# liamhebert/MultiModalDiscussionTransformer

Measured on AMD Instinct MI355X. Metric: discussion-tree comments/sec fwd+bwd, higher is better.
Workload: dtype bf16; 1 GPU; mDT-base (BERT-base + ViT-B/16 split 6+6, 6 executed graph layers, D768 H12 nb4 L100), 32 bushy 64-comment trees per GPU, 25% image comments, random-init weights, dropout 0.4/0.3/0.3 (run_train.sh:37), token lengths U{8..100} zero-padded to 100 (SURVEY.md §8d; mean 54.3 valid tokens), text side ragged: padded token positions are not computed (identical logits / gradients), last fusion layer comput; trees_per_gpu=32, parallelism=dp1, frozen_initial_encoders=False

## Files before the change

multimodaldiscussiontransformer_amd/csrc/common.hpp:

```cpp
#pragma once
#include <hip/hip_runtime.h>
#include <stdint.h>
#include <stdio.h>
#include <string.h>

#include <atomic>

#include "../../include/mdt_hip.h"

namespace mdt {

constexpr int WAVE = 64;

typedef __bf16 bf16_t;
typedef __attribute__((ext_vector_type(8))) __bf16 bf16x8;
typedef __attribute__((ext_vector_type(4))) __bf16 bf16x4;
typedef __attribute__((ext_vector_type(2))) __bf16 bf16x2;
typedef __attribute__((ext_vector_type(4))) float f32x4;
typedef __attribute__((ext_vector_type(2))) float f32x2;
typedef __attribute__((ext_vector_type(4))) short s16x4;
typedef __attribute__((ext_vector_type(4))) int i32x4;

void set_error(const char* fmt, ...);
#define MDT_CHECK_ARG(cond, ...)          \
  do {                                    \
    if (!(cond)) {                        \
      ::mdt::set_error(__VA_ARGS__);      \
      return MDT_ERR_ARG;                 \
    }                                     \
  } while (0)
#define MDT_UNSUPPORTED(...)              \
  do {                                    \
    ::mdt::set_error(__VA_ARGS__);        \
    return MDT_ERR_UNSUPPORTED;           \
  } while (0)
int check_launch(const char* what);

enum class GemmRoute { none, generic, tile128, tile256x128, pp256, pp256p, w4p, w4s };
inline constexpr const char* GEMM_ROUTE_NAMES[] = {"", "generic", "tile128", "tile256x128", "pp256", "pp256p", "w4p", "w4s"};
enum class AttnRoute { none, v1, v2, v3, v4, v4x, v5, long_ };
inline constexpr const char* ATTN_ROUTE_NAMES[] = {"", "v1", "v2", "v3", "v4", "v4x", "v5", "long"};
inline const char* route_name(GemmRoute r) { return GEMM_ROUTE_NAMES[(int)r]; }
inline const char* route_name(AttnRoute r) { return ATTN_ROUTE_NAMES[(int)r]; }

struct Switches {
  GemmRoute gemm_route;
  bool gemm_dynamic;
  bool gemm_stamp;
  int gemm_diag;
  int gemm_f8w;
  AttnRoute attn_bwd;
  bool ln_generic;
  int ln_bwd_wgs;
};
const Switches& switches();
int device_cus();

void set_last_route(const char* route);
template <auto Kern, typename... Args>
int launch_route(const char* route, dim3 grid, dim3 block, size_t lds, hipStream_t st, Args... args) {
  static std::atomic<size_t> raised{64 * 1024};
  if (lds > raised.load(std::memory_order_relaxed)) {
    if (hipFuncSetAttribute((const void*)Kern, hipFuncAttributeMaxDynamicSharedMemorySize, (int)lds) != hipSuccess) {
      (void)hipGetLastError();
      set_error("%s: cannot reserve %zu bytes of LDS", route, lds);
      return MDT_ERR_LAUNCH;
    }
    raised.store(lds, std::memory_order_relaxed);
  }
  hipLaunchKernelGGL(Kern, grid, block, lds, st, args...);
  if (int e = check_launch(route)) return e;
  set_last_route(route);
  return MDT_OK;
}

template <typename T> __device__ __forceinline__ float to_f32(T v);
template <> __device__ __forceinline__ float to_f32<float>(float v) { return v; }
template <> __device__ __forceinline__ float to_f32<bf16_t>(bf16_t v) { return (float)v; }
template <typename T> __device__ __forceinline__ T from_f32(float v);
template <> __device__ __forceinline__ float from_f32<float>(float v) { return v; }
template <> __device__ __forceinline__ bf16_t from_f32<bf16_t>(float v) { return (bf16_t)v; }

__device__ __forceinline__ float wave_sum(float v) {
#pragma unroll
  for (int o = 32; o > 0; o >>= 1) v += __shfl_xor(v, o, 64);
  return v;
}
__device__ __forceinline__ float wave_max(float v) {
#pragma unroll
  for (int o = 32; o > 0; o >>= 1) v = fmaxf(v, __shfl_xor(v, o, 64));
  return v;
}
__device__ __forceinline__ float quad16_sum(float v) {
  v += __shfl_xor(v, 16, 64);
  v += __shfl_xor(v, 32, 64);
  return v;
}
__device__ __forceinline__ float row16_sum(float v) {
#pragma unroll
  for (int o = 8; o > 0; o >>= 1) v += __shfl_xor(v, o, 64);
  return v;
}
__device__ __forceinline__ float row16_sum_dpp(float v) {
  v += __builtin_bit_cast(float, __builtin_amdgcn_mov_dpp(__builtin_bit_cast(int, v), 0x128, 0xf, 0xf, true));
  v += __builtin_bit_cast(float, __builtin_amdgcn_mov_dpp(__builtin_bit_cast(int, v), 0x124, 0xf, 0xf, true));
  v += __builtin_bit_cast(float, __builtin_amdgcn_mov_dpp(__builtin_bit_cast(int, v), 0x122, 0xf, 0xf, true));
  v += __builtin_bit_cast(float, __builtin_amdgcn_mov_dpp(__builtin_bit_cast(int, v), 0x121, 0xf, 0xf, true));
  return v;
}
__device__ __forceinline__ float wave_sum_dpp(float v) {
  v = row16_sum_dpp(v);
  v += __builtin_bit_cast(float, __builtin_amdgcn_update_dpp(0, __builtin_bit_cast(int, v), 0x142, 0xa, 0xf, false));
  v += __builtin_bit_cast(float, __builtin_amdgcn_update_dpp(0, __builtin_bit_cast(int, v), 0x143, 0xc, 0xf, false));
  return __builtin_bit_cast(float, __builtin_amdgcn_readlane(__builtin_bit_cast(int, v), 63));
}
__device__ __forceinline__ float row16_max(float v) {
#pragma unroll
  for (int o = 8; o > 0; o >>= 1) v = fmaxf(v, __shfl_xor(v, o, 64));
  return v;
}

__device__ __forceinline__ float gelu_erf(float x) { return 0.5f * x * (1.0f + erff(x * 0.70710678118654752f)); }
__device__ __forceinline__ float gelu_erf_grad(float x) {
  const float cdf = 0.5f * (1.0f + erff(x * 0.70710678118654752f));
  const float pdf = 0.3989422804014327f * __expf(-0.5f * x * x);
  return cdf + x * pdf;
}

__device__ __forceinline__ void gelu_fast_parts(float x, float& cdf, float& pdf) {
  const float z = fabsf(x) * 0.70710678118654752f;
  const float t = __builtin_amdgcn_rcpf(__builtin_fmaf(0.3275911f, z, 1.0f));
  const float e = __builtin_amdgcn_exp2f(z * z * -1.4426950408889634f);
  float poly = __builtin_fmaf(t, 1.061405429f, -1.453152027f);
  poly = __builtin_fmaf(t, poly, 1.421413741f);
  poly = __builtin_fmaf(t, poly, -0.284496736f);
  poly = __builtin_fmaf(t, poly, 0.254829592f);
  const float erf_abs = __builtin_fmaf(-(poly * t), e, 1.0f);
  cdf = __builtin_fmaf(0.5f, copysignf(erf_abs, x), 0.5f);
  pdf = 0.3989422804014327f * e;
}
__device__ __forceinline__ float gelu_fast(float x) {
  float cdf, pdf;
  gelu_fast_parts(x, cdf, pdf);
  return x * cdf;
}
__device__ __forceinline__ float gelu_fast_grad(float x) {
  float cdf, pdf;
  gelu_fast_parts(x, cdf, pdf);
  return cdf + x * pdf;
}

__device__ __forceinline__ uint32_t drop_mix(uint32_t x) {
  x = __umul24(x, 0x95F24Du) + __builtin_rotateleft32(x, 15); x ^= x >> 15;
  x = __umul24(x, 0xC2B2AEu) + __builtin_rotateleft32(x, 13); x ^= x >> 13;
  x = __umul24(x, 0x85EBCBu) + __builtin_rotateleft32(x, 17); x ^= x >> 16;
  return x;
}
struct DropCfg {
  uint32_t key;
  uint32_t thresh;
  float inv_keep;
};
__device__ __forceinline__ float drop_scale(const DropCfg& d, uint64_t idx) {
  const uint32_t h = drop_mix((uint32_t)(idx >> 1) ^ d.key);
  const uint32_t bits = (idx & 1) ? (h >> 16) : (h & 0xFFFFu);
  return bits >= d.thresh ? d.inv_keep : 0.f;
}
__device__ __forceinline__ void drop_scale2(const DropCfg& d, uint64_t idx_even, float& s0, float& s1) {
  const uint32_t h = drop_mix((uint32_t)(idx_even >> 1) ^ d.key);
  s0 = (h & 0xFFFFu) >= d.thresh ? d.inv_keep : 0.f;
  s1 = (h >> 16) >= d.thresh ? d.inv_keep : 0.f;
}
constexpr int64_t DROP_MAX_ELEMS = (int64_t)1 << 33;
static inline DropCfg make_drop(float p, uint64_t seed) {
  DropCfg d;
  uint64_t z = seed + 0x9E3779B97F4A7C15ull;
  z = (z ^ (z >> 30)) * 0xBF58476D1CE4E5B9ull;
  z = (z ^ (z >> 27)) * 0x94D049BB133111EBull;
  z ^= z >> 31;
  d.key = (uint32_t)(z ^ (z >> 32));
  d.thresh = (uint32_t)(p * 65536.0f + 0.5f);
  d.inv_keep = 1.0f / (1.0f - p);
  return d;
}

__device__ __forceinline__ f32x4 mfma_f32(float a, float b, f32x4 c) {
  return __builtin_amdgcn_mfma_f32_16x16x4f32(a, b, c, 0, 0, 0);
}
__device__ __forceinline__ f32x4 mfma_bf16(bf16x8 a, bf16x8 b, f32x4 c) {
  return __builtin_amdgcn_mfma_f32_16x16x32_bf16(a, b, c, 0, 0, 0);
}

#define LDS_PTR(p) ((__attribute__((address_space(3))) void*)(p))

__device__ __forceinline__ bf16x4 lds_read_tr16(const bf16_t* lds_addr) {
  typedef __attribute__((address_space(3))) s16x4* lds_s16x4_ptr;
  s16x4 r = __builtin_amdgcn_ds_read_tr16_b64_v4i16((lds_s16x4_ptr)(lds_addr));
  return __builtin_bit_cast(bf16x4, r);
}

__device__ __forceinline__ void glds16(const void* gptr, void* lds_wave_base) {
  __builtin_amdgcn_global_load_lds((const __attribute__((address_space(1))) void*)gptr,
// ... 11 lines not shown
```

multimodaldiscussiontransformer_amd/csrc/gemm.hip:

```cpp
#include <stdlib.h>

#include <algorithm>
#include <type_traits>
#include <vector>

#include "common.hpp"
#include "gemm_tiles.hpp"
#include "gemm_epilogue.hpp"

namespace mdt {

template <typename TIn, typename TOut, bool TA, bool TB>
__global__ __launch_bounds__(256) void gemm_generic_kernel(GemmParams p) {
  constexpr int BM = 64, BN = 64, BK = 16, LD = 68;
  __shared__ float As[BK][LD];
  __shared__ float Bs[BK][LD];
  const int tid = threadIdx.x, lane = tid & 63, wave = tid >> 6;
  const int wr = wave >> 1, wc = wave & 1;
  const int64_t m0 = (int64_t)blockIdx.y * BM, n0 = (int64_t)blockIdx.x * BN;
  const int64_t kbeg = (int64_t)blockIdx.z * p.k_chunk;
  const int64_t kend = (kbeg + p.k_chunk < p.K) ? kbeg + p.k_chunk : p.K;
  const TIn* A = (const TIn*)p.A;
  const TIn* B = (const TIn*)p.B;
  f32x4 acc[2][2];
#pragma unroll
  for (int i = 0; i < 2; ++i)
#pragma unroll
    for (int j = 0; j < 2; ++j) acc[i][j] = f32x4{0.f, 0.f, 0.f, 0.f};

  for (int64_t k0 = kbeg; k0 < kend; k0 += BK) {
#pragma unroll
    for (int i = 0; i < 4; ++i) {
      const int e = tid + i * 256;
      int r, k;
      if constexpr (!TA) { r = e >> 4; k = e & 15; } else { k = e >> 6; r = e & 63; }
      const int64_t gr = m0 + r, gk = k0 + k;
      float v = 0.f;
      if (gr < p.M && gk < kend) v = to_f32(TA ? A[gk * p.lda + gr] : A[gr * p.lda + gk]);
      As[k][r] = v;
      int c, kb;
      if constexpr (!TB) { c = e >> 4; kb = e & 15; } else { kb = e >> 6; c = e & 63; }
      const int64_t gc = n0 + c, gkb = k0 + kb;
      float w = 0.f;
      if (gc < p.N && gkb < kend) w = to_f32(TB ? B[gkb * p.ldb + gc] : B[gc * p.ldb + gkb]);
      Bs[kb][c] = w;
    }
    __syncthreads();
#pragma unroll
    for (int kk = 0; kk < BK; kk += 4) {
      float a[2], b[2];
#pragma unroll
      for (int i = 0; i < 2; ++i) a[i] = As[kk + (lane >> 4)][wr * 32 + i * 16 + (lane & 15)];
#pragma unroll
      for (int j = 0; j < 2; ++j) b[j] = Bs[kk + (lane >> 4)][wc * 32 + j * 16 + (lane & 15)];
#pragma unroll
      for (int i = 0; i < 2; ++i)
#pragma unroll
        for (int j = 0; j < 2; ++j) acc[i][j] = mfma_f32(a[i], b[j], acc[i][j]);
    }
    __syncthreads();
  }
#pragma unroll
  for (int i = 0; i < 2; ++i)
#pragma unroll
    for (int j = 0; j < 2; ++j)
#pragma unroll
      for (int r = 0; r < 4; ++r)
        epilogue_store<TIn, TOut>(p, m0 + wr * 32 + i * 16 + (lane >> 4) * 4 + r,
                                  n0 + wc * 32 + j * 16 + (lane & 15), acc[i][j][r]);
}

template <typename TOut, bool A_KM, bool B_KM>
__global__ __launch_bounds__(256) void gemm_bf16_tile128(GemmParams p) {
  extern __shared__ __attribute__((aligned(16))) char smem[];
  const int tid = threadIdx.x;
  const int lane = tid & 63;
  const int wave = __builtin_amdgcn_readfirstlane(tid >> 6);
  const int wr = wave >> 1, wc = wave & 1;

  const int nwg = p.tiles_m * p.tiles_n;
  const int bid = blockIdx.x;
  const int q8 = nwg >> 3, r8 = nwg & 7, xcd = bid & 7;
  const int tile = (xcd < r8 ? xcd * (q8 + 1) : r8 * (q8 + 1) + (xcd - r8) * q8) + (bid >> 3);
  const int tm = tile / p.tiles_n, tn = tile - tm * p.tiles_n;
  const int64_t m0 = (int64_t)tm * T_BM, n0 = (int64_t)tn * T_BN;
  const int64_t kbeg = (int64_t)blockIdx.z * p.k_chunk;
  const int64_t kend = (kbeg + p.k_chunk < p.K) ? kbeg + p.k_chunk : p.K;
  const int nk = (int)((kend - kbeg + T_BK - 1) / T_BK);

  const int64_t lda_b = p.lda * 2, ldb_b = p.ldb * 2;
  const char* a_base;
  const char* b_base;
  int64_t a_bytes, b_bytes;
  if constexpr (!A_KM) { a_base = (const char*)p.A + m0 * lda_b; a_bytes = (p.M - m0) * lda_b; }
  else { a_base = (const char*)p.A + kbeg * lda_b; a_bytes = (kend - kbeg) * lda_b; }
  if constexpr (!B_KM) { b_base = (const char*)p.B + n0 * ldb_b; b_bytes = (p.N - n0) * ldb_b; }
  else { b_base = (const char*)p.B + kbeg * ldb_b; b_bytes = (kend - kbeg) * ldb_b; }
  const unsigned a_rec = (unsigned)(a_bytes > 0xFFFFFFF0ll ? 0xFFFFFFF0ll : a_bytes);
  const unsigned b_rec = (unsigned)(b_bytes > 0xFFFFFFF0ll ? 0xFFFFFFF0ll : b_bytes);
  const __amdgpu_buffer_rsrc_t rsA = __builtin_amdgcn_make_buffer_rsrc((void*)a_base, 0, a_rec, 0x00020000);
  const __amdgpu_buffer_rsrc_t rsB = __builtin_amdgcn_make_buffer_rsrc((void*)b_base, 0, b_rec, 0x00020000);
  const int64_t a_k0 = A_KM ? 0 : kbeg, b_k0 = B_KM ? 0 : kbeg;
  const int a_col0 = A_KM ? (int)m0 : 0, b_col0 = B_KM ? (int)n0 : 0;

  f32x4 acc[4][4];
#pragma unroll
  for (int i = 0; i < 4; ++i)
#pragma unroll
    for (int j = 0; j < 4; ++j) acc[i][j] = f32x4{0.f, 0.f, 0.f, 0.f};

  if (nk > 0) {
    stage_tile<A_KM, 128, 4>(rsA, lda_b, a_k0, a_col0, smem, wave, lane);
    stage_tile<B_KM, 128, 4>(rsB, ldb_b, b_k0, b_col0, smem + T_TILE_BYTES, wave, lane);
  }
  for (int kt = 0; kt < nk; ++kt) {
    char* cur = smem + (kt & 1) * 2 * T_TILE_BYTES;
    char* nxt = smem + ((kt + 1) & 1) * 2 * T_TILE_BYTES;
    __syncthreads();
    if (kt + 1 < nk) {
      stage_tile<A_KM, 128, 4>(rsA, lda_b, a_k0 + (int64_t)(kt + 1) * T_BK, a_col0, nxt, wave, lane);
      stage_tile<B_KM, 128, 4>(rsB, ldb_b, b_k0 + (int64_t)(kt + 1) * T_BK, b_col0, nxt + T_TILE_BYTES, wave, lane);
    }
#pragma unroll
    for (int ks = 0; ks < 2; ++ks) {
      bf16x8 a[4], b[4];
#pragma unroll
      for (int i = 0; i < 4; ++i) a[i] = load_frag<A_KM, 128>(cur, wr * 64 + i * 16, ks, lane);
#pragma unroll
      for (int j = 0; j < 4; ++j) b[j] = load_frag<B_KM, 128>(cur + T_TILE_BYTES, wc * 64 + j * 16, ks, lane);
#pragma unroll
      for (int i = 0; i < 4; ++i)
#pragma unroll
        for (int j = 0; j < 4; ++j) acc[i][j] = mfma_bf16(a[i], b[j], acc[i][j]);
    }
  }
  tile_epilogue<TOut>(p, acc, smem, wave, lane, m0 + wr * 64, n0 + wc * 64);
}

template <typename TOut, bool A_KM, bool B_KM, int BN, int WM, int WN, int NSTAGE>
__global__ __launch_bounds__(512) void gemm_bf16_tile256(GemmParams p) {
  constexpr int BM = 256;
  constexpr int MI = BM / WM / 16, NI = BN / WN / 16;
  constexpr int A_BYTES = BM * 128, B_BYTES = BN * 128, STAGE = A_BYTES + B_BYTES;
  constexpr int LOADS = (BM + BN) / 64;
  extern __shared__ __attribute__((aligned(16))) char smem[];
  const int tid = threadIdx.x;
  const int lane = tid & 63;
  const int wave = __builtin_amdgcn_readfirstlane(tid >> 6);
  const int wr = wave / WN, wc = wave % WN;

  const int nwg = p.tiles_m * p.tiles_n;
  const int bid = blockIdx.x;
  const int q8 = nwg >> 3, r8 = nwg & 7, xcd = bid & 7;
  const int tile = (xcd < r8 ? xcd * (q8 + 1) : r8 * (q8 + 1) + (xcd - r8) * q8) + (bid >> 3);
  const int tm = tile / p.tiles_n, tn = tile - tm * p.tiles_n;
  const int64_t m0 = (int64_t)tm * BM, n0 = (int64_t)tn * BN;
  const int64_t kbeg = (int64_t)blockIdx.z * p.k_chunk;
  const int64_t kend = (kbeg + p.k_chunk < p.K) ? kbeg + p.k_chunk : p.K;
  const int nk = (int)((kend - kbeg + T_BK - 1) / T_BK);

  const int64_t lda_b = p.lda * 2, ldb_b = p.ldb * 2;
  const char* a_base;
  const char* b_base;
  int64_t a_bytes, b_bytes;
  if constexpr (!A_KM) { a_base = (const char*)p.A + m0 * lda_b; a_bytes = (p.M - m0) * lda_b; }
  else { a_base = (const char*)p.A + kbeg * lda_b; a_bytes = (kend - kbeg) * lda_b; }
  if constexpr (!B_KM) { b_base = (const char*)p.B + n0 * ldb_b; b_bytes = (p.N - n0) * ldb_b; }
  else { b_base = (const char*)p.B + kbeg * ldb_b; b_bytes = (kend - kbeg) * ldb_b; }
  const unsigned a_rec = (unsigned)(a_bytes > 0xFFFFFFF0ll ? 0xFFFFFFF0ll : a_bytes);
  const unsigned b_rec = (unsigned)(b_bytes > 0xFFFFFFF0ll ? 0xFFFFFFF0ll : b_bytes);
  const __amdgpu_buffer_rsrc_t rsA = __builtin_amdgcn_make_buffer_rsrc((void*)a_base, 0, a_rec, 0x00020000);
  const __amdgpu_buffer_rsrc_t rsB = __builtin_amdgcn_make_buffer_rsrc((void*)b_base, 0, b_rec, 0x00020000);
  const int64_t a_k0 = A_KM ? 0 : kbeg, b_k0 = B_KM ? 0 : kbeg;
  const int a_col0 = A_KM ? (int)m0 : 0, b_col0 = B_KM ? (int)n0 : 0;

  f32x4 acc[MI][NI];
#pragma unroll
  for (int i = 0; i < MI; ++i)
#pragma unroll
    for (int j = 0; j < NI; ++j) acc[i][j] = f32x4{0.f, 0.f, 0.f, 0.f};

  auto issue = [&](int kt) {
    char* st = smem + (kt % NSTAGE) * STAGE;
    stage_tile<A_KM, BM, 8>(rsA, lda_b, a_k0 + (int64_t)kt * T_BK, a_col0, st, wave, lane);
    stage_tile<B_KM, BN, 8>(rsB, ldb_b, b_k0 + (int64_t)kt * T_BK, b_col0, st + A_BYTES, wave, lane);
  };
#pragma unroll
  for (int s = 0; s < NSTAGE - 1; ++s)
    if (nk > s) issue(s);
  for (int kt = 0; kt < nk; ++kt) {
    if (NSTAGE == 3 && kt + 1 < nk) {
      if constexpr (LOADS == 6) asm volatile("s_waitcnt vmcnt(6)" ::: "memory");
      else asm volatile("s_waitcnt vmcnt(8)" ::: "memory");
    } else {
      asm volatile("s_waitcnt vmcnt(0)" ::: "memory");
    }
    __builtin_amdgcn_s_barrier();
    if (kt + NSTAGE - 1 < nk) issue(kt + NSTAGE - 1);
    const char* cur = smem + (kt % NSTAGE) * STAGE;
#pragma unroll
    for (int ks = 0; ks < 2; ++ks) {
      bf16x8 a[MI], b[NI];
#pragma unroll
      for (int j = 0; j < NI; ++j) b[j] = load_frag<B_KM, BN>(cur + A_BYTES, wc * (NI * 16) + j * 16, ks, lane);
#pragma unroll
      for (int i = 0; i < MI; ++i) a[i] = load_frag<A_KM, BM>(cur, wr * (MI * 16) + i * 16, ks, lane);
#pragma unroll
      for (int i = 0; i < MI; ++i)
#pragma unroll
        for (int j = 0; j < NI; ++j) acc[i][j] = mfma_bf16(a[i], b[j], acc[i][j]);
    }
  }
#pragma unroll
  for (int h = 0; h < MI / 4; ++h) {
    f32x4 blk[4][4];
#pragma unroll
    for (int i = 0; i < 4; ++i)
#pragma unroll
      for (int j = 0; j < 4; ++j) blk[i][j] = acc[h * 4 + i][j];
    tile_epilogue<TOut>(p, blk, smem, wave, lane, m0 + wr * (MI * 16) + h * 64, n0 + wc * 64);
  }
}

constexpr int pp_nb(int dist) { return dist + 1 < 4 ? 4 : dist + 1; }

template <typename TOut, bool A_KM, bool B_KM, int PP_DIST>
__global__ __launch_bounds__(512) void gemm_bf16_pp256(GemmParams p) {
  constexpr int PP_NB = pp_nb(PP_DIST);
  constexpr int BM = 256, BN = 256;
  constexpr int A_BYTES = BM * 64;
  constexpr bool SWAP = sizeof(TOut) == 2;
  extern __shared__ __attribute__((aligned(16))) char smem[];
  const int tid = threadIdx.x;
  const int lane = tid & 63;
  const int wave = __builtin_amdgcn_readfirstlane(tid >> 6);
  const int wr = wave >> 2, wc = wave & 3;
  const bool late = wave >= 4;

  const int tiles = p.tiles_m * p.tiles_n;
  const int nwg = tiles * (int)gridDim.z;
  const int bid = (int)blockIdx.z * (int)gridDim.x + (int)blockIdx.x;
  const int q8 = nwg >> 3, r8 = nwg & 7, xcd = bid & 7;
  const int work = (xcd < r8 ? xcd * (q8 + 1) : r8 * (q8 + 1) + (xcd - r8) * q8) + (bid >> 3);
  const int slab = work / tiles;
  const int tile = work - slab * tiles;
  int tm, tn;
  {
    const int G = p.group_n, per_group = p.tiles_m * G;
    const int gi = tile / per_group;
    const int full = p.tiles_n / G;
    if (gi < full) {
      const int r = tile - gi * per_group;
      tm = r / G;
      tn = gi * G + (r - tm * G);
    } else {
      const int gsz = p.tiles_n - full * G;
      const int r = tile - full * per_group;
      tm = r / gsz;
      tn = full * G + (r - tm * gsz);
    }
  }
  const int64_t m0 = (int64_t)tm * BM, n0 = (int64_t)tn * BN;
  const int64_t kbeg = (int64_t)slab * p.k_chunk;
  const int64_t kend = (kbeg + p.k_chunk < p.K) ? kbeg + p.k_chunk : p.K;
  const int nk = (int)((kend - kbeg + T_BK - 1) / T_BK);
  const int nhs = 2 * nk;

  const int64_t lda_b = p.lda * 2, ldb_b = p.ldb * 2;
  const char* a_base;
  const char* b_base;
  int64_t a_bytes, b_bytes;
  if constexpr (!A_KM) { a_base = (const char*)p.A + m0 * lda_b; a_bytes = (p.M - m0) * lda_b; }
  else { a_base = (const char*)p.A + kbeg * lda_b; a_bytes = (kend - kbeg) * lda_b; }
  if constexpr (!B_KM) { b_base = (const char*)p.B + n0 * ldb_b; b_bytes = (p.N - n0) * ldb_b; }
  else { b_base = (const char*)p.B + kbeg * ldb_b; b_bytes = (kend - kbeg) * ldb_b; }
  const unsigned a_rec = (unsigned)(a_bytes > 0xFFFFFFF0ll ? 0xFFFFFFF0ll : a_bytes);
  const unsigned b_rec = (unsigned)(b_bytes > 0xFFFFFFF0ll ? 0xFFFFFFF0ll : b_bytes);
  const __amdgpu_buffer_rsrc_t rsA = __builtin_amdgcn_make_buffer_rsrc((void*)a_base, 0, a_rec, 0x00020000);
  const __amdgpu_buffer_rsrc_t rsB = __builtin_amdgcn_make_buffer_rsrc((void*)b_base, 0, b_rec, 0x00020000);
  const int64_t a_k0 = A_KM ? 0 : kbeg, b_k0 = B_KM ? 0 : kbeg;
  const int a_col0 = A_KM ? (int)m0 : 0, b_col0 = B_KM ? (int)n0 : 0;

  f32x4 acc[8][4];
#pragma unroll
  for (int i = 0; i < 8; ++i)
#pragma unroll
    for (int j = 0; j < 4; ++j) acc[i][j] = f32x4{0.f, 0.f, 0.f, 0.f};
// ... 704 lines not shown
  std::sort(cyc.begin(), cyc.end());
  std::sort(clk.begin(), clk.end());
  fprintf(stderr, "[mdt gemm stamp] M=%lld N=%lld K=%lld wgs=%zu  cycles/k-tile median %.0f (p10 %.0f p90 %.0f)  clock median %.0f MHz  span %.1f us\n",
          (long long)p.M, (long long)p.N, (long long)p.K, nwg, cyc[cyc.size() / 2], cyc[cyc.size() / 10], cyc[cyc.size() * 9 / 10],
          clk[clk.size() / 2], (double)(t1 - t0) / 100.0);
  std::vector<unsigned long long> st(256);
  if (hipMemcpy(st.data(), dev + nwg * 4, 256 * 8, hipMemcpyDeviceToHost) == hipSuccess && st[0]) {
    fprintf(stderr, "[mdt gemm steps]");
    for (int i = 1; i < 256 && st[i]; ++i) fprintf(stderr, " %llu", st[i] - st[i - 1]);
    fprintf(stderr, "\n");
  } else (void)hipGetLastError();
}

static int num_cus() {
  const int n = device_cus() & ~7;
  return n < 8 ? 8 : n;
}

static int* g_tile_queues = nullptr;
static int g_tile_queue_sets = 0;

static int xcd_group_n(int tiles_m, int tiles_n, double b_panel, int n_cus) {
  if (tiles_n % 2 == 0 && b_panel * tiles_n > 3.5e6 && b_panel * (tiles_n / 2) <= 2.5e6 && (double)tiles_m * tiles_n >= 4.0 * n_cus)
    return tiles_n / 2;
  return tiles_n;
}

struct GemmPlan {
  GemmRoute route;
  int tiles_m, tiles_n, split_k, group_n;
  int64_t k_chunk;
  dim3 grid;
  bool strip_asum;
};

static GemmPlan plan_gemm(const GemmParams& p, int dtype, int out_dtype, int ta, int tb, int n_cus) {
  const Switches& sw = switches();
  const int64_t M = p.M, N = p.N, K = p.K;
  const int epi = p.epilogue;
  bool fast = dtype == MDT_BF16 && K > 0 && (ta ? M % T_BM == 0 : K % T_BK == 0) && (tb ? N % T_BN == 0 : K % T_BK == 0) &&
              N % T_BN == 0 && p.lda % 8 == 0 && p.ldb % 8 == 0 && ((uintptr_t)p.A | (uintptr_t)p.B) % 16 == 0 &&
              p.lda * 2 * 128 < (1ll << 31) && p.ldb * 2 * 128 < (1ll << 31);
  const int ov = out_dtype == MDT_F32 ? 4 : 8;
  if (!(epi & MDT_EPI_ATOMIC) && (p.ldc % ov || ((uintptr_t)p.C & 15))) fast = false;
  if ((epi & MDT_EPI_BIAS) && ((uintptr_t)p.bias & 15)) fast = false;
  if ((epi & MDT_EPI_RESIDUAL) && (p.ldr % 8 || ((uintptr_t)p.residual & 15))) fast = false;
  if (p.aux && (p.ldaux % 8 || ((uintptr_t)p.aux & 15))) fast = false;
  const int64_t chunk = ((K + p.split_k - 1) / p.split_k + T_BK - 1) / T_BK * T_BK;
  if (fast && (ta || tb) && chunk * (ta ? p.lda : p.ldb) * 2 >= (1ll << 32)) fast = false;
  const int split = fast ? (int)((K + chunk - 1) / chunk) : 1;

  const bool m256 = ta ? M % 256 == 0 : true;
  const int tm256 = (int)((M + 255) / 256), tn256 = (int)(N / 256);
  const bool pp = fast && m256 && N % 256 == 0;
  const int nhs = 2 * (int)((K + T_BK - 1) / T_BK);
  auto persist = [&](int min_steps) {
    return pp && out_dtype == MDT_BF16 && split == 1 && nhs >= min_steps && tm256 * tn256 > n_cus;
  };
  const bool queue = sw.gemm_dynamic && g_tile_queues;
  auto ok = [&](GemmRoute r) {
    switch (r) {
      case GemmRoute::generic: return true;
      case GemmRoute::tile128: return fast;
      case GemmRoute::tile256x128: return fast && m256;
      case GemmRoute::pp256: return pp;
      case GemmRoute::pp256p: return persist(4);
      case GemmRoute::w4p:
        return persist(16) && nhs >= W4_NEXPL + 2 && !queue && !(epi & (1 << 24));
      case GemmRoute::w4s:
        return pp && out_dtype == MDT_F32 && !sw.gemm_stamp && (epi & MDT_EPI_ATOMIC) &&
               !(epi & ((1 << 20) - 1) & ~(MDT_EPI_ATOMIC | MDT_EPI_ASUM)) && chunk >= 256 && K - (int64_t)(split - 1) * chunk >= 256;
      default: return false;
    }
  };
  GemmRoute r;
  const int64_t t256 = (int64_t)tm256 * (N / 128) * split;
  if (!fast) r = GemmRoute::generic;
  else if (pp && t256 / 2 >= 200) {
    const int e = epi & ((1 << 22) - 1);
    const bool light = e == 0 || e == MDT_EPI_BIAS || e == MDT_EPI_RESIDUAL || e == (MDT_EPI_BIAS | MDT_EPI_RESIDUAL | MDT_EPI_DROPOUT) ||
                       e == (MDT_EPI_MULAUX | MDT_EPI_COLSUM);
    if (persist(16)) r = ok(GemmRoute::w4p) && !ta && light ? GemmRoute::w4p : GemmRoute::pp256p;
    else r = ok(GemmRoute::w4s) ? GemmRoute::w4s : GemmRoute::pp256;
  } else if (m256 && t256 >= 256) r = GemmRoute::tile256x128;
  else r = GemmRoute::tile128;
  if (sw.gemm_route != GemmRoute::none && ok(sw.gemm_route)) r = sw.gemm_route;

  GemmPlan pl{};
  pl.route = r;
  pl.group_n = 1 << 30;
  pl.strip_asum = r != GemmRoute::pp256 && r != GemmRoute::w4s;
  if (r == GemmRoute::generic) {
    const int64_t c16 = ((K + p.split_k - 1) / p.split_k + 15) / 16 * 16;
    pl.k_chunk = c16 < 16 ? 16 : c16;
    pl.split_k = K > 0 ? (int)((K + pl.k_chunk - 1) / pl.k_chunk) : 1;
    pl.grid = dim3((unsigned)((N + 63) / 64), (unsigned)((M + 63) / 64), (unsigned)pl.split_k);
    return pl;
  }
  pl.k_chunk = chunk;
  pl.split_k = split;
  pl.tiles_m = r == GemmRoute::tile128 ? (int)((M + T_BM - 1) / T_BM) : tm256;
  pl.tiles_n = r == GemmRoute::tile128 || r == GemmRoute::tile256x128 ? (int)(N / T_BN) : tn256;
  pl.grid = dim3((unsigned)(pl.tiles_m * pl.tiles_n), 1, (unsigned)split);
  if (r == GemmRoute::tile128 || r == GemmRoute::tile256x128) return pl;
  pl.group_n = split > 1 ? (pl.tiles_n > pl.tiles_m ? 1 : pl.tiles_n) : xcd_group_n(pl.tiles_m, pl.tiles_n, 256.0 * (double)chunk * 2.0, n_cus);
  if (r == GemmRoute::pp256p || r == GemmRoute::w4p) pl.grid.x = (unsigned)n_cus;
  return pl;
}

constexpr int E_BIAS = MDT_EPI_BIAS, E_DENSE = MDT_EPI_BIAS | MDT_EPI_RESIDUAL | MDT_EPI_DROPOUT,
              E_FC1 = MDT_EPI_BIAS | MDT_EPI_GELU | MDT_EPI_AUX_GRAD , E_RES = MDT_EPI_RESIDUAL,
              E_DFC2 = MDT_EPI_MULAUX | MDT_EPI_COLSUM;
template <int E> using EpiK = std::integral_constant<int, E>;
template <bool A_KM, bool B_KM, class F>
static int with_epilogue(const GemmParams& p, F&& f) {
  const int e = p.epilogue & ((1 << 22) - 1);
  if constexpr (!A_KM && !B_KM) {
    if (e == E_BIAS) return f(EpiK<E_BIAS>{});
    if (e == E_DENSE) return f(EpiK<E_DENSE>{});
    if (e == E_FC1 && p.aux) return f(EpiK<E_FC1>{});
  }
  if constexpr (!A_KM) {
    if (e == 0) return f(EpiK<0>{});
    if (e == E_RES) return f(EpiK<E_RES>{});
    if (e == E_DFC2) return f(EpiK<E_DFC2>{});
  }
  return f(EpiK<-1>{});
}

template <class F>
static int with_layout(int ta, int tb, F&& f) {
  using T = std::true_type;
  using N = std::false_type;
  if (!ta && !tb) return f(N{}, N{});
  if (!ta) return f(N{}, T{});
  if (!tb) return f(T{}, N{});
  return f(T{}, T{});
}

template <typename TIn, typename TOut>
static int launch_generic(hipStream_t st, const GemmParams& p, dim3 grid, int ta, int tb) {
  return with_layout(ta, tb, [&](auto a_t, auto b_t) {
    return launch_route<gemm_generic_kernel<TIn, TOut, decltype(a_t)::value, decltype(b_t)::value>>("generic", grid, 256, 0, st, p);
  });
}

template <typename TOut>
static int launch_gemm(hipStream_t st, const GemmParams& p, GemmRoute r, dim3 grid, int ta, int tb) {
  const size_t pp_lds = (size_t)pp_nb(4) * PP_STAGE;
  const char* name = route_name(r);
  return with_layout(ta, tb, [&](auto a_km, auto b_km) -> int {
    constexpr bool A = decltype(a_km)::value, B = decltype(b_km)::value;
    switch (r) {
      case GemmRoute::tile128: return launch_route<gemm_bf16_tile128<TOut, A, B>>(name, grid, 256, 4 * T_TILE_BYTES, st, p);
      case GemmRoute::tile256x128:
        return launch_route<gemm_bf16_tile256<TOut, A, B, 128, 4, 2, 3>>(name, grid, 512, (size_t)3 * (256 + 128) * 128, st, p);
      case GemmRoute::pp256: return launch_route<gemm_bf16_pp256<TOut, A, B, 4>>(name, grid, 512, pp_lds, st, p);
      case GemmRoute::w4p:
        return with_epilogue<A, B>(p, [&](auto ek) {
          return launch_route<gemm_bf16_w4p<A, B, decltype(ek)::value>>(name, grid, 256, (size_t)5 * PP_STAGE, st, p);
        });
      case GemmRoute::pp256p:
        return with_epilogue<A, B>(p, [&](auto ek) {
          constexpr int EPK = decltype(ek)::value;
          if (!(p.epilogue & (1 << 24))) return launch_route<gemm_bf16_pp256p<A, B, 4, EPK>>(name, grid, 512, pp_lds, st, p);
          constexpr int EJ = (!B && (EPK == E_FC1 || EPK == E_DENSE)) || (B && EPK == E_DFC2) ? EPK : -1;
          return launch_route<gemm_bf16_pp256p<A, B, 4, EJ, 0, true>>(name, grid, 512, pp_lds, st, p);
        });
      default: set_error("mdt_gemm: route %s has no launch here", name); return MDT_ERR_ARG;
    }
  });
}

template <int F8>
static int launch_pp256p_f8(hipStream_t st, const GemmParams& p) {
  const int nvt = p.tiles_m * p.tiles_n;
  const dim3 grid((unsigned)(nvt < num_cus() ? nvt : num_cus()), 1, 1);
  const size_t lds = (size_t)pp_nb(4) * PP_STAGE;
  const int e = p.epilogue;
#define LF8(E_) return launch_route<gemm_bf16_pp256p<false, false, 4, E_, F8>>("f8_pp256p", grid, 512, lds, st, p)
  if constexpr (F8 == 1) {
    if (e == E_BIAS) LF8(E_BIAS);
    if (e == E_DENSE) LF8(E_DENSE);
    if (e == E_FC1 && p.aux) LF8(E_FC1);
  } else {
    if (e == 0) LF8(0);
    if (e == E_RES) LF8(E_RES);
    if (e == E_DFC2) LF8(E_DFC2);
  }
  LF8(-1);
#undef LF8
}

}

using namespace mdt;

extern "C" int mdt_gemm(void* stream, int dtype, int out_dtype, int trans_a, int trans_b, int64_t M, int64_t N,
                        int64_t K, const void* A, int64_t lda, const void* B, int64_t ldb, void* C, int64_t ldc,
                        int epilogue, float alpha, const void* bias, const void* residual, int64_t ldr, void* aux,
                        int64_t ldaux, int split_k, float drop_p, uint64_t drop_seed, float* colsum) {
  MDT_CHECK_ARG(dtype == MDT_F32 || dtype == MDT_BF16, "mdt_gemm: bad dtype %d", dtype);
  MDT_CHECK_ARG(out_dtype == MDT_F32 || out_dtype == MDT_BF16, "mdt_gemm: bad out_dtype %d", out_dtype);
  MDT_CHECK_ARG(M >= 0 && N >= 0 && K >= 0, "mdt_gemm: negative shape");
  if (M == 0 || N == 0) return MDT_OK;
  MDT_CHECK_ARG(A && B && C, "mdt_gemm: null operand");
  MDT_CHECK_ARG(!(epilogue & MDT_EPI_BIAS) || bias, "mdt_gemm: MDT_EPI_BIAS without bias");
  MDT_CHECK_ARG(!(epilogue & MDT_EPI_RESIDUAL) || residual, "mdt_gemm: MDT_EPI_RESIDUAL without residual");
  MDT_CHECK_ARG(!(epilogue & (MDT_EPI_DGELU | MDT_EPI_MULAUX)) || aux, "mdt_gemm: MDT_EPI_DGELU / MDT_EPI_MULAUX without aux");
  MDT_CHECK_ARG(!(epilogue & MDT_EPI_AUX_GRAD) || (epilogue & MDT_EPI_GELU), "mdt_gemm: MDT_EPI_AUX_GRAD needs MDT_EPI_GELU");
  MDT_CHECK_ARG(!(epilogue & MDT_EPI_ATOMIC) || out_dtype == MDT_F32, "mdt_gemm: MDT_EPI_ATOMIC needs fp32 C");
  MDT_CHECK_ARG(dtype == MDT_BF16 || out_dtype == MDT_F32, "mdt_gemm: fp32 inputs need fp32 output");
  if (split_k < 1) split_k = 1;
  MDT_CHECK_ARG(split_k == 1 || (epilogue & MDT_EPI_ATOMIC), "mdt_gemm: split_k > 1 needs MDT_EPI_ATOMIC");
  MDT_CHECK_ARG(!(epilogue & MDT_EPI_DROPOUT) || (drop_p >= 0.f && drop_p < 1.f), "mdt_gemm: dropout p=%f out of [0,1)", drop_p);
  MDT_CHECK_ARG(split_k == 1 || !(epilogue & (MDT_EPI_BIAS | MDT_EPI_GELU | MDT_EPI_RESIDUAL | MDT_EPI_DGELU | MDT_EPI_DROPOUT | MDT_EPI_MULAUX)),
                "mdt_gemm: split_k > 1 supports only the plain accumulate epilogue");
  hipStream_t st = (hipStream_t)stream;
  GemmParams p;
  p.M = M; p.N = N; p.K = K; p.A = A; p.lda = lda; p.B = B; p.ldb = ldb; p.C = C; p.ldc = ldc;
  p.epilogue = epilogue; p.alpha = alpha; p.bias = bias; p.residual = residual; p.ldr = ldr;
  p.aux = aux; p.ldaux = ldaux; p.split_k = split_k;
  MDT_CHECK_ARG(!(epilogue & MDT_EPI_DROPOUT) || M * N < DROP_MAX_ELEMS, "mdt_gemm: dropout site of %lld elements (limit 2^33)", (long long)(M * N));
  p.drop = make_drop((epilogue & MDT_EPI_DROPOUT) ? drop_p : 0.f, drop_seed);
  p.colsum = colsum;
  p.stamps = nullptr;
  p.tile_queue = nullptr;
  p.alpha_dev = p.alpha_dev2 = nullptr;
  p.epilogue |= switches().gemm_diag << 20;
  MDT_CHECK_ARG(!(epilogue & MDT_EPI_COLSUM) || (colsum && split_k == 1), "mdt_gemm: MDT_EPI_COLSUM needs a colsum buffer and split_k == 1");
  MDT_CHECK_ARG(!(epilogue & MDT_EPI_ASUM) || (colsum && trans_a && (epilogue & MDT_EPI_ATOMIC) && !(epilogue & MDT_EPI_COLSUM) && dtype == MDT_BF16 && out_dtype == MDT_F32),
                "mdt_gemm: MDT_EPI_ASUM needs bf16 operands, an fp32 C, trans_a = 1, MDT_EPI_ATOMIC, a colsum buffer and no MDT_EPI_COLSUM");
  const GemmPlan pl = plan_gemm(p, dtype, out_dtype, trans_a, trans_b, num_cus());
  p.k_chunk = pl.k_chunk; p.split_k = pl.split_k; p.tiles_m = pl.tiles_m; p.tiles_n = pl.tiles_n; p.group_n = pl.group_n;
  if (pl.strip_asum && (p.epilogue & MDT_EPI_ASUM)) {
    p.epilogue &= ~MDT_EPI_ASUM;
    if (int e = mdt_colsum(stream, dtype, K, M, A, lda, colsum, nullptr)) return e;
  }
  switch (pl.route) {
    case GemmRoute::generic:
      if (dtype == MDT_F32) return launch_generic<float, float>(st, p, pl.grid, trans_a, trans_b);
      return out_dtype == MDT_F32 ? launch_generic<bf16_t, float>(st, p, pl.grid, trans_a, trans_b)
                                  : launch_generic<bf16_t, bf16_t>(st, p, pl.grid, trans_a, trans_b);
    case GemmRoute::w4s: return launch_w4s(st, p, pl.grid, trans_a, trans_b);
    case GemmRoute::pp256p:
      if (switches().gemm_dynamic && g_tile_queues) {
        static unsigned turn = 0;
        p.tile_queue = g_tile_queues + 16 * (turn++ % (unsigned)g_tile_queue_sets);
      }
      [[fallthrough]];
    case GemmRoute::pp256:
      if (switches().gemm_stamp) {
        const size_t bytes = (size_t)pl.grid.x * pl.grid.z * 32 + 256 * 8;
        if (hipMalloc(&p.stamps, bytes) != hipSuccess) { (void)hipGetLastError(); p.stamps = nullptr; }
        else (void)hipMemsetAsync(p.stamps, 0, bytes, st);
      }
      break;
    default: break;
  }
  const int e = out_dtype == MDT_F32 ? launch_gemm<float>(st, p, pl.route, pl.grid, trans_a, trans_b)
                                     : launch_gemm<bf16_t>(st, p, pl.route, pl.grid, trans_a, trans_b);
  if (p.stamps) {
    if (e == MDT_OK) report_stamps(p.stamps, (size_t)pl.grid.x * pl.grid.z, p);
    (void)hipFree(p.stamps);
  }
  return e;
}

extern "C" size_t mdt_gemm_tile_queue_bytes(void) { return (size_t)512 * 16 * sizeof(int); }

extern "C" int mdt_gemm_set_tile_queue(void* zeroed_device_buffer, size_t bytes) {
  if (zeroed_device_buffer == nullptr) { g_tile_queues = nullptr; g_tile_queue_sets = 0; return MDT_OK; }
  MDT_CHECK_ARG(bytes >= 16 * sizeof(int) && ((uintptr_t)zeroed_device_buffer & 3) == 0, "mdt_gemm_set_tile_queue: buffer too small / unaligned");
  g_tile_queues = (int*)zeroed_device_buffer;
  g_tile_queue_sets = (int)(bytes / (16 * sizeof(int)));
  return MDT_OK;
}

extern "C" int mdt_gemm_fp8(void* stream, int a_format, int64_t M, int64_t N, int64_t K, const void* A, int64_t lda,
                            const void* B, int64_t ldb, void* C, int64_t ldc, int epilogue, const float* inv_scale_a,
                            const float* inv_scale_b, const void* bias, const void* residual, int64_t ldr, void* aux,
                            int64_t ldaux, float drop_p, uint64_t drop_seed, float* colsum) {
  return mdt_gemm_fp8_q8(stream, a_format, M, N, K, A, lda, B, ldb, C, ldc, epilogue, inv_scale_a, inv_scale_b, bias, residual, ldr,
                         aux, ldaux, drop_p, drop_seed, colsum, nullptr, 0, 0, nullptr, nullptr);
}

extern "C" int mdt_gemm_fp8_q8(void* stream, int a_format, int64_t M, int64_t N, int64_t K, const void* A, int64_t lda,
                               const void* B, int64_t ldb, void* C, int64_t ldc, int epilogue, const float* inv_scale_a,
                               const float* inv_scale_b, const void* bias, const void* residual, int64_t ldr, void* aux,
                               int64_t ldaux, float drop_p, uint64_t drop_seed, float* colsum, void* q8_out, int64_t ld_q8,
                               int q8_format, const float* q8_scale, float* q8_amax) {
  MDT_CHECK_ARG(a_format == 0 || a_format == 1, "mdt_gemm_fp8: a_format %d (0 = e4m3, 1 = e5m2)", a_format);
  MDT_CHECK_ARG(M >= 0 && N >= 0 && K >= 0, "mdt_gemm_fp8: negative shape");
  if (M == 0 || N == 0) return MDT_OK;
  MDT_CHECK_ARG(A && B && C && inv_scale_a && inv_scale_b, "mdt_gemm_fp8: null operand / scale");
  MDT_CHECK_ARG(!(epilogue & MDT_EPI_BIAS) || bias, "mdt_gemm_fp8: MDT_EPI_BIAS without bias");
  MDT_CHECK_ARG(!(epilogue & MDT_EPI_RESIDUAL) || residual, "mdt_gemm_fp8: MDT_EPI_RESIDUAL without residual");
  MDT_CHECK_ARG(!(epilogue & (MDT_EPI_DGELU | MDT_EPI_MULAUX)) || aux, "mdt_gemm_fp8: MDT_EPI_DGELU / MDT_EPI_MULAUX without aux");
  MDT_CHECK_ARG(!(epilogue & MDT_EPI_AUX_GRAD) || (epilogue & MDT_EPI_GELU), "mdt_gemm_fp8: MDT_EPI_AUX_GRAD needs MDT_EPI_GELU");
  MDT_CHECK_ARG(!(epilogue & (MDT_EPI_ATOMIC | MDT_EPI_ACCUM)), "mdt_gemm_fp8: bf16 store epilogues only");
  MDT_CHECK_ARG(!(epilogue & MDT_EPI_COLSUM) || colsum, "mdt_gemm_fp8: MDT_EPI_COLSUM needs a colsum buffer");
  MDT_CHECK_ARG(!(epilogue & MDT_EPI_DROPOUT) || (drop_p >= 0.f && drop_p < 1.f && M * N < DROP_MAX_ELEMS), "mdt_gemm_fp8: bad dropout site");
  const bool ok = N % 256 == 0 && K % 64 == 0 && K >= 256 && lda % 16 == 0 && ldb % 16 == 0 && (((uintptr_t)A | (uintptr_t)B) % 16 == 0) &&
                  ldc % 8 == 0 && ((uintptr_t)C & 15) == 0 && (!(epilogue & MDT_EPI_BIAS) || ((uintptr_t)bias & 15) == 0) &&
                  (!(epilogue & MDT_EPI_RESIDUAL) || (ldr % 8 == 0 && ((uintptr_t)residual & 15) == 0)) &&
                  (!aux || (ldaux % 8 == 0 && ((uintptr_t)aux & 15) == 0)) && lda * 256 < (1ll << 31) && ldb * 256 < (1ll << 31);
  if (!ok) MDT_UNSUPPORTED("mdt_gemm_fp8: shape M=%lld N=%lld K=%lld (needs N %% 256 == 0, K %% 64 == 0, K >= 256, 16-byte rows)",
// ... 105 lines not shown
```

multimodaldiscussiontransformer_amd/csrc/host.cpp:

```cpp
#include <stdarg.h>
#include <stdlib.h>
#include <string.h>

#include <algorithm>
#include <cmath>
#include <limits>
#include <vector>

#include "common.hpp"

namespace mdt {

static thread_local char g_err[512] = "";

void set_error(const char* fmt, ...) {
  va_list ap;
  va_start(ap, fmt);
  vsnprintf(g_err, sizeof(g_err), fmt, ap);
  va_end(ap);
}

int check_launch(const char* what) {
  hipError_t e = hipGetLastError();
  if (e != hipSuccess) {
    set_error("%s: launch failed: %s", what, hipGetErrorString(e));
    return MDT_ERR_LAUNCH;
  }
  return MDT_OK;
}

static thread_local const char* g_route = "";
void set_last_route(const char* route) { g_route = route; }

static Switches g_sw;
static bool g_sw_valid = false;

template <size_t N>
static int pick(const char* var, const char* const (&names)[N]) {
  const char* v = getenv(var);
  if (!v || !*v) return 0;
  for (size_t i = 1; i < N; ++i)
    if (!strcmp(v, names[i])) return (int)i;
  fprintf(stderr, "[mdt] %s=%s names no route: the default routes run\n", var, v);
  return 0;
}

static void read_switches() {
  auto flag = [](const char* n) { return getenv(n) != nullptr; };
  auto num = [](const char* n, int dflt) { const char* v = getenv(n); return v ? atoi(v) : dflt; };
  g_sw.gemm_route = (GemmRoute)pick("MDT_GEMM_ROUTE", GEMM_ROUTE_NAMES);
  g_sw.gemm_dynamic = num("MDT_GEMM_DYNAMIC", 0) != 0;
  g_sw.gemm_stamp = flag("MDT_GEMM_STAMP");
  g_sw.gemm_diag = num("MDT_GEMM_DIAG", 0);
  g_sw.gemm_f8w = num("MDT_GEMM_F8W", 1);
  g_sw.attn_bwd = (AttnRoute)pick("MDT_ATTN_BWD", ATTN_ROUTE_NAMES);
  g_sw.ln_generic = flag("MDT_LN_GENERIC");
  g_sw.ln_bwd_wgs = num("MDT_LN_BWD_WGS", 2048);
  g_sw_valid = true;
}

const Switches& switches() {
  if (!g_sw_valid) read_switches();
  return g_sw;
}

int device_cus() {
  static int n = 0;
  if (!n) {
    int dev = 0;
    hipDeviceProp_t prop;
    if (hipGetDevice(&dev) == hipSuccess && hipGetDeviceProperties(&prop, dev) == hipSuccess) n = prop.multiProcessorCount;
    if (n <= 0) n = 256;
  }
  return n;
}

}

extern "C" void mdt_reload_env(void) { mdt::read_switches(); }
extern "C" int mdt_abi_version(void) { return MDT_ABI_VERSION; }
extern "C" const char* mdt_last_error_string(void) { return mdt::g_err; }
extern "C" const char* mdt_last_route(void) { return mdt::g_route; }

namespace {

struct SpatialTable {
  int t[6][6];
  SpatialTable() {
    std::vector<int> vals;
    for (int a = 0; a < 6; ++a)
      for (int b = a; b < 6; ++b) vals.push_back((a + b) * (a + b + 1) / 2 + a);
    std::sort(vals.begin(), vals.end());
    for (int a = 0; a < 6; ++a)
      for (int b = 0; b < 6; ++b) {
        const int lo = std::min(a, b), hi = std::max(a, b);
        const int c = (lo + hi) * (lo + hi + 1) / 2 + lo;
        t[a][b] = (int)(std::lower_bound(vals.begin(), vals.end(), c) - vals.begin());
      }
  }
};
const SpatialTable kTable;

}

extern "C" int mdt_pack_structure_ud(int B, const int64_t* n_nodes, const int64_t* const* parents,
                                     const int64_t* const* updown, int nmax, int spatial_pos_max, float* attn_bias,
                                     int32_t* spatial_pos, int64_t* in_degree) {
  MDT_CHECK_ARG(B >= 0 && nmax >= 1 && n_nodes && parents && attn_bias && spatial_pos && in_degree,
                "pack_structure: bad arguments");
  const int T = nmax + 1;
  const float ninf = -std::numeric_limits<float>::infinity();
  std::vector<int> depth, anc_pos;
  for (int b = 0; b < B; ++b) {
    const int n = (int)n_nodes[b];
    const int64_t* par = parents[b];
    MDT_CHECK_ARG(n >= 1 && n <= nmax, "pack_structure: tree %d has %d nodes (nmax %d)", b, n, nmax);
    float* ab = attn_bias + (int64_t)b * T * T;
    int32_t* sp = spatial_pos + (int64_t)b * nmax * nmax;
    int64_t* deg = in_degree + (int64_t)b * nmax;
    depth.assign(n, 0);
    for (int i = 0; i < n; ++i) {
      MDT_CHECK_ARG(par[i] < i && par[i] >= -1 && (i == 0) == (par[i] < 0),
                    "pack_structure: tree %d node %d: parents must precede children (root first)", b, i);
      depth[i] = par[i] < 0 ? 0 : depth[par[i]] + 1;
    }
    for (int i = 0; i < T; ++i)
      for (int j = 0; j < T; ++j) ab[(int64_t)i * T + j] = (j <= n) ? 0.f : ninf;
    std::fill(sp, sp + (int64_t)nmax * nmax, 0);
    std::fill(deg, deg + nmax, (int64_t)0);
    for (int i = 0; i < n; ++i) {
      deg[i] += 1;
      if (par[i] >= 0) { deg[i] += 1; deg[par[i]] += 1; }
    }
    for (int i = 0; i < n; ++i) {
      for (int j = 0; j < n; ++j) {
        int up = 0, down = 0;
        if (updown && updown[b]) {
          const int64_t* e = updown[b] + ((int64_t)i * n + j) * 2;
          MDT_CHECK_ARG(e[0] >= 0 && e[1] >= 0 && e[0] < (1 << 20) && e[1] < (1 << 20), "pack_structure: tree %d: negative hop count", b);
          up = (int)e[0];
          down = (int)e[1];
        } else {
          int a = i, c = j;
          while (a != c) {
            if (depth[a] >= depth[c]) { a = (int)par[a]; ++up; }
            else { c = (int)par[c]; ++down; }
          }
        }
        const int bucket = (up <= 5 && down <= 5) ? kTable.t[up][down] : kTable.t[5][5];
        sp[(int64_t)i * nmax + j] = bucket + 1;
        if (up + down >= spatial_pos_max) ab[(int64_t)(i + 1) * T + (j + 1)] = ninf;
      }
    }
  }
  return MDT_OK;
}

extern "C" int mdt_pack_structure(int B, const int64_t* n_nodes, const int64_t* const* parents, int nmax,
                                  int spatial_pos_max, float* attn_bias, int32_t* spatial_pos, int64_t* in_degree) {
  return mdt_pack_structure_ud(B, n_nodes, parents, nullptr, nmax, spatial_pos_max, attn_bias, spatial_pos, in_degree);
}

extern "C" int mdt_resize_plan_ksize(int in_size, int out_size) {
  if (in_size <= 0 || out_size <= 0) return 0;
  double filterscale = (double)in_size / (double)out_size;
  if (filterscale < 1.0) filterscale = 1.0;
  const double support = 1.0 * filterscale;
  return (int)ceil(support) * 2 + 1;
}

extern "C" int mdt_resize_plan(int in_size, int out_size, int32_t* bounds, int32_t* coeffs, int ksize) {
  MDT_CHECK_ARG(in_size > 0 && out_size > 0 && bounds && coeffs, "mdt_resize_plan: bad arguments");
  MDT_CHECK_ARG(ksize == mdt_resize_plan_ksize(in_size, out_size), "mdt_resize_plan: ksize %d, expected %d", ksize,
                mdt_resize_plan_ksize(in_size, out_size));
  const double scale = (double)in_size / (double)out_size;
  double filterscale = scale;
  if (filterscale < 1.0) filterscale = 1.0;
  const double support = 1.0 * filterscale;
  const double ss = 1.0 / filterscale;
  std::vector<double> k((size_t)ksize);
  for (int xx = 0; xx < out_size; ++xx) {
    const double center = 0.0 + (xx + 0.5) * scale;
    double ww = 0.0;
    int xmin = (int)(center - support + 0.5);
    if (xmin < 0) xmin = 0;
    int xmax = (int)(center + support + 0.5);
    if (xmax > in_size) xmax = in_size;
    xmax -= xmin;
    for (int x = 0; x < xmax; ++x) {
      double t = (x + xmin - center + 0.5) * ss;
      if (t < 0.0) t = -t;
      const double w = t < 1.0 ? 1.0 - t : 0.0;
      k[x] = w;
      ww += w;
    }
    for (int x = 0; x < xmax; ++x)
      if (ww != 0.0) k[x] /= ww;
    int32_t* kk = coeffs + (size_t)xx * ksize;
    for (int x = 0; x < ksize; ++x) {
      const double v = x < xmax ? k[x] : 0.0;
      kk[x] = v < 0 ? (int32_t)(-0.5 + v * (double)(1 << 22)) : (int32_t)(0.5 + v * (double)(1 << 22));
    }
    bounds[2 * xx] = xmin;
    bounds[2 * xx + 1] = xmax;
  }
  return MDT_OK;
// ... 12 lines not shown
```

Measured before the change: 16100 comments/s.

## Add 4-stage BK=32 ring pipeline to tile128 GEMM for K-major layouts

Adds a multi-stage ring-buffered K loop to the 128x128 GEMM kernel. It issues global-to-LDS loads for stage s+3 while computing stage s, using 32-wide K slices and counted vmem waits. By default the 4-stage variant runs whenever either operand is K-major, and the original double-buffered path stays for the NN layout. An environment switch can force either variant. This tries to hide global load latency better, but it adds more barriers and smaller MFMA batches per step.

```diff
diff --git a/multimodaldiscussiontransformer_amd/csrc/common.hpp b/multimodaldiscussiontransformer_amd/csrc/common.hpp
--- a/multimodaldiscussiontransformer_amd/csrc/common.hpp
+++ b/multimodaldiscussiontransformer_amd/csrc/common.hpp
@@ -48,6 +48,7 @@
   bool gemm_dynamic;
   bool gemm_stamp;
   int gemm_diag;
+  int gemm_t128_stages;
   int gemm_f8w;
   AttnRoute attn_bwd;
   bool ln_generic;
diff --git a/multimodaldiscussiontransformer_amd/csrc/gemm.hip b/multimodaldiscussiontransformer_amd/csrc/gemm.hip
--- a/multimodaldiscussiontransformer_amd/csrc/gemm.hip
+++ b/multimodaldiscussiontransformer_amd/csrc/gemm.hip
@@ -70,7 +70,28 @@
                                   n0 + wc * 32 + j * 16 + (lane & 15), acc[i][j][r]);
 }
 
-template <typename TOut, bool A_KM, bool B_KM>
+template <bool KM>
+__device__ __forceinline__ bf16x8 ring_frag(const char* lds_tile, int rc_base, int lane) {
+  if constexpr (KM) return w4_frag<true, 128>(lds_tile, rc_base, lane);
+  else return load_frag_h<false, 128>(lds_tile, rc_base, lane);
+}
+
+template <bool KM>
+__device__ __forceinline__ void ring_frag_wait(bf16x8 (&f)[4]) {
+  if constexpr (KM) asm volatile("s_waitcnt lgkmcnt(0)" : "+v"(f[0]), "+v"(f[1]), "+v"(f[2]), "+v"(f[3]) : : "memory");
+}
+
+template <int MAXA, int LOADS>
+__device__ __forceinline__ void wait_ring(int ahead) {
+  if constexpr (MAXA > 0) {
+    if (ahead >= MAXA) wait_vm<MAXA * LOADS>();
+    else wait_ring<MAXA - 1, LOADS>(ahead);
+  } else {
+    wait_vm<0>();
+  }
+}
+
+template <typename TOut, bool A_KM, bool B_KM, int NSTAGE = 2>
 __global__ __launch_bounds__(256) void gemm_bf16_tile128(GemmParams p) {
   extern __shared__ __attribute__((aligned(16))) char smem[];
   const int tid = threadIdx.x;
@@ -109,6 +130,39 @@
 #pragma unroll
     for (int j = 0; j < 4; ++j) acc[i][j] = f32x4{0.f, 0.f, 0.f, 0.f};
 
+  if constexpr (NSTAGE > 2) {
+    constexpr int BK = 32, OP_BYTES = 128 * BK * 2, STAGE = 2 * OP_BYTES;
+    constexpr int LOADS = STAGE / 4096;
+    const int ns = nk * (T_BK / BK);
+    auto issue = [&](int s, int slot) {
+      char* st = smem + slot * STAGE;
+      stage_step<A_KM, 128, 4>(rsA, lda_b, a_k0 + (int64_t)s * BK, a_col0, st, wave, lane);
+      stage_step<B_KM, 128, 4>(rsB, ldb_b, b_k0 + (int64_t)s * BK, b_col0, st + OP_BYTES, wave, lane);
+    };
+#pragma unroll
+    for (int s = 0; s < NSTAGE - 1; ++s)
+      if (s < ns) issue(s, s);
+    int cur = 0, nxt = NSTAGE - 1;
+    for (int s = 0; s < ns; ++s) {
+      wait_ring<NSTAGE - 2, LOADS>(ns - 1 - s);
+      __builtin_amdgcn_s_barrier();
+      if (s + NSTAGE - 1 < ns) issue(s + NSTAGE - 1, nxt);
+      const char* st = smem + cur * STAGE;
+      bf16x8 a[4], b[4];
+#pragma unroll
+      for (int i = 0; i < 4; ++i) a[i] = ring_frag<A_KM>(st, wr * 64 + i * 16, lane);
+#pragma unroll
+      for (int j = 0; j < 4; ++j) b[j] = ring_frag<B_KM>(st + OP_BYTES, wc * 64 + j * 16, lane);
+      ring_frag_wait<A_KM>(a);
+      ring_frag_wait<B_KM>(b);
+#pragma unroll
+      for (int i = 0; i < 4; ++i)
+#pragma unroll
+        for (int j = 0; j < 4; ++j) acc[i][j] = mfma_bf16(a[i], b[j], acc[i][j]);
+      cur = cur + 1 == NSTAGE ? 0 : cur + 1;
+      nxt = nxt + 1 == NSTAGE ? 0 : nxt + 1;
+    }
+  } else {
   if (nk > 0) {
     stage_tile<A_KM, 128, 4>(rsA, lda_b, a_k0, a_col0, smem, wave, lane);
     stage_tile<B_KM, 128, 4>(rsB, ldb_b, b_k0, b_col0, smem + T_TILE_BYTES, wave, lane);
@@ -133,6 +187,7 @@
 #pragma unroll
         for (int j = 0; j < 4; ++j) acc[i][j] = mfma_bf16(a[i], b[j], acc[i][j]);
     }
+  }
   }
   tile_epilogue<TOut>(p, acc, smem, wave, lane, m0 + wr * 64, n0 + wc * 64);
 }
@@ -1143,7 +1198,11 @@
   return with_layout(ta, tb, [&](auto a_km, auto b_km) -> int {
     constexpr bool A = decltype(a_km)::value, B = decltype(b_km)::value;
     switch (r) {
-      case GemmRoute::tile128: return launch_route<gemm_bf16_tile128<TOut, A, B>>(name, grid, 256, 4 * T_TILE_BYTES, st, p);
+      case GemmRoute::tile128: {
+        const int ts = switches().gemm_t128_stages;
+        if (ts == 2 || (ts != 4 && !A && !B)) return launch_route<gemm_bf16_tile128<TOut, A, B>>(name, grid, 256, 4 * T_TILE_BYTES, st, p);
+        return launch_route<gemm_bf16_tile128<TOut, A, B, 4>>(name, grid, 256, 4 * T_TILE_BYTES, st, p);
+      }
       case GemmRoute::tile256x128:
         return launch_route<gemm_bf16_tile256<TOut, A, B, 128, 4, 2, 3>>(name, grid, 512, (size_t)3 * (256 + 128) * 128, st, p);
       case GemmRoute::pp256: return launch_route<gemm_bf16_pp256<TOut, A, B, 4>>(name, grid, 512, pp_lds, st, p);
diff --git a/multimodaldiscussiontransformer_amd/csrc/host.cpp b/multimodaldiscussiontransformer_amd/csrc/host.cpp
--- a/multimodaldiscussiontransformer_amd/csrc/host.cpp
+++ b/multimodaldiscussiontransformer_amd/csrc/host.cpp
@@ -52,6 +52,7 @@
   g_sw.gemm_dynamic = num("MDT_GEMM_DYNAMIC", 0) != 0;
   g_sw.gemm_stamp = flag("MDT_GEMM_STAMP");
   g_sw.gemm_diag = num("MDT_GEMM_DIAG", 0);
+  g_sw.gemm_t128_stages = num("MDT_GEMM_T128_STAGES", 0);
   g_sw.gemm_f8w = num("MDT_GEMM_F8W", 1);
   g_sw.attn_bwd = (AttnRoute)pick("MDT_ATTN_BWD", ATTN_ROUTE_NAMES);
   g_sw.ln_generic = flag("MDT_LN_GENERIC");
```

Result: no change. 16170 comments/s (median of 6 runs) (+0.4%).
